# devsisters/libquic

Measured on AMD Instinct MI355X. Metric: FEC XOR encode+recover GiB/s (device-resident) on batched 1350B packet groups, higher is better.
Workload: dtype u8; 1 GPU; 1048576 groups x 10 x 1350 B per GPU: parity encode + single-loss recover (BASELINE configs[1]+[2]); groups_per_gpu=1048576, k=10, L=1350, parallelism=group-shard x1 (no collective)

## Files before the change

libquic_amd/csrc/qfec_kernels.hip:

```cpp
#include "qfec_internal.h"

#include <algorithm>
#include <type_traits>
#include <cstdlib>

namespace qfec {
namespace {

typedef uint32_t u32x4 __attribute__((ext_vector_type(4)));

constexpr uint32_t kMaxPacket = 1452;
constexpr int kBlock = 256;

__device__ __forceinline__ u32x4 ld16(const uint8_t* p) {
  u32x4 v;
  __builtin_memcpy(&v, p, 16);
  return v;
}

template <bool NT>
__device__ __forceinline__ u32x4 ld16t(const uint8_t* p) {
  if constexpr (NT) {
    return __builtin_nontemporal_load(reinterpret_cast<const u32x4*>(p));
  } else {
    return ld16(p);
  }
}

__device__ __forceinline__ void st16(uint8_t* p, u32x4 v) { __builtin_memcpy(p, &v, 16); }

template <bool NT>
__device__ __forceinline__ void st16t(uint8_t* p, u32x4 v) {
  if constexpr (NT) {
    __builtin_nontemporal_store(v, reinterpret_cast<u32x4*>(p));
  } else {
    st16(p, v);
  }
}

__device__ __forceinline__ uint32_t wave_max11(uint32_t v) {
  uint32_t mx = 0;
#pragma unroll
  for (int b = 10; b >= 0; --b) {
    const uint32_t cand = mx | (1u << b);
    if (__ballot(v >= cand) != 0ull) mx = cand;
  }
  return mx;
}

__device__ __forceinline__ bool wave_any(bool p) { return __ballot(p) != 0ull; }

template <int N, bool RECOVER, bool NT>
__device__ __forceinline__ void xor_rows_n(u32x4& acc, const uint8_t* src, uint64_t row_stride,
                                           uint32_t r, uint32_t m, const uint8_t* par) {
  u32x4 v[N];
#pragma unroll
  for (int w = 0; w < N; ++w) {
    const uint8_t* q = (RECOVER && r + (uint32_t)w == m) ? par : src + (uint64_t)(r + w) * row_stride;
    v[w] = ld16t<NT>(q);
  }
#pragma unroll
  for (int w = 0; w < N; ++w) acc ^= v[w];
}

template <int B, bool RECOVER, bool NT>
__device__ __forceinline__ void xor_rows_rt(u32x4& acc, const uint8_t* src, uint64_t row_stride,
                                            uint32_t k, uint32_t m, const uint8_t* par) {
  static_assert(B == 8 || B == 16 || B == 32, "batch of 8, 16 or 32 rows");
  const uint32_t nb = (k + B - 1) / B;
  const uint32_t base = nb ? k / nb : 0u, extra = k - base * nb;
  uint32_t r = 0;
  for (uint32_t b = 0; b < nb; ++b) {
    const uint32_t n = base + (b < extra ? 1u : 0u);
#define QFEC_REM(N)                                                 \
  case N:                                                           \
    xor_rows_n<N, RECOVER, NT>(acc, src, row_stride, r, m, par);    \
    break;
    if (B == 8 || n <= 8u) {
      switch (n) {
        QFEC_REM(1) QFEC_REM(2) QFEC_REM(3) QFEC_REM(4) QFEC_REM(5) QFEC_REM(6) QFEC_REM(7)
        QFEC_REM(8)
        default:
          break;
      }
    } else if constexpr (B >= 16) {
      if (B == 16 || n <= 16u) {
        switch (n) {
          QFEC_REM(9) QFEC_REM(10) QFEC_REM(11) QFEC_REM(12) QFEC_REM(13) QFEC_REM(14)
          QFEC_REM(15) QFEC_REM(16)
          default:
            break;
        }
      } else if constexpr (B == 32) {
        switch (n) {
          QFEC_REM(17) QFEC_REM(18) QFEC_REM(19) QFEC_REM(20) QFEC_REM(21) QFEC_REM(22)
          QFEC_REM(23) QFEC_REM(24) QFEC_REM(25) QFEC_REM(26) QFEC_REM(27) QFEC_REM(28)
          QFEC_REM(29) QFEC_REM(30) QFEC_REM(31) QFEC_REM(32)
          default:
            break;
        }
      }
    }
#undef QFEC_REM
    r += n;
  }
}

template <int KC, bool RECOVER, bool NT, bool SM, bool INPL = false>
__global__ __launch_bounds__(kBlock) void fixed_xor_kernel(FixedArgs a, uint32_t C,
                                                           uint32_t gpb) {
  static_assert(!(INPL && RECOVER), "in place: the encode form over the k rows");
  const uint32_t tid = threadIdx.x;
  const uint32_t gl = tid / C;
  const uint32_t t = tid - gl * C;
  const uint64_t gb = (uint64_t)blockIdx.x * gpb;
  const uint64_t g = gb + gl;
  if constexpr (INPL) {
    const bool on = gl < gpb && g < a.n_groups;
    const uint64_t gg = on ? g : 0;
    const uint32_t off = min(t * 16u, a.L - 16u);
    const uint8_t* src = a.rows + gg * a.group_stride + off;
    const uint32_t k = KC > 0 ? (uint32_t)KC : a.k;
    const uint32_t m = on ? (uint32_t)a.inplace_missing[gg] : 0u;
    u32x4 acc = {0u, 0u, 0u, 0u};
    if constexpr (KC > 0) {
      xor_rows_n<(KC > 0 ? KC : 1), false, NT>(acc, src, a.row_stride, 0, 0, nullptr);
    } else {
      xor_rows_rt<8, false, NT>(acc, src, a.row_stride, k, 0, nullptr);
    }
    __syncthreads();
    if (on && m < k) st16t<NT>(const_cast<uint8_t*>(src) + (uint64_t)m * a.row_stride, acc);
    if (on && m >= k && t == 0) atomicOr(a.err, kErrMissingIndex);
    return;
  }
  uint64_t mw0 = 0, mw1 = 0;
  if constexpr (RECOVER) {
    if constexpr (SM) {
      const uint8_t* mp = a.missing + gb;
      const uint32_t mis = (uint32_t)((uintptr_t)mp & 7u);
      const uint64_t* wp = reinterpret_cast<const uint64_t*>(mp - mis);
      mw0 = wp[0];
      if (gb + 8u - mis < a.n_groups) mw1 = wp[1];
    }
  }
  if (gl >= gpb || g >= a.n_groups) return;
  const uint32_t off = min(t * 16u, a.L - 16u);
  const uint8_t* src = a.rows + g * a.group_stride + off;
  const uint32_t k = KC > 0 ? (uint32_t)KC : a.k;

  u32x4 acc = {0u, 0u, 0u, 0u};
  if constexpr (RECOVER) {
    uint32_t m;
    if constexpr (SM) {
      const uint32_t sh = gl + (uint32_t)((uintptr_t)(a.missing + gb) & 7u);
      m = (uint32_t)((sh < 8u ? mw0 >> (8u * sh) : mw1 >> (8u * (sh - 8u))) & 0xFFu);
    } else {
      m = a.missing[g];
    }
    if (m >= k) {
      if (t == 0) atomicOr(a.err, kErrMissingIndex);
      return;
    }
    const uint8_t* par = a.parity + g * a.parity_stride + off;
    if constexpr (KC > 0) {
#pragma unroll
      for (uint32_t i = 0; i < (uint32_t)KC; ++i) {
        const uint8_t* p = (i == m) ? par : src + i * a.row_stride;
        acc ^= ld16t<NT>(p);
      }
    } else {
      xor_rows_rt<8, true, NT>(acc, src, a.row_stride, k, m, par);
    }
  } else {
    if constexpr (KC > 0) {
#pragma unroll
      for (uint32_t i = 0; i < (uint32_t)KC; ++i) acc ^= ld16t<NT>(src + i * a.row_stride);
    } else {
      xor_rows_rt<8, false, NT>(acc, src, a.row_stride, k, 0, nullptr);
    }
  }
  st16t<NT>(a.out + g * a.out_stride + off, acc);
}

constexpr int kPhSteps = 40;
constexpr int kPhRegSteps = 32;
constexpr uint64_t kPhTimeout = 20000;

__device__ __forceinline__ uint32_t* ph_word(uint32_t* ps, uint32_t i) { return ps + 64u * i; }

__device__ __forceinline__ uint32_t ph_load(uint32_t* w) {
  return __hip_atomic_load(w, __ATOMIC_RELAXED, __HIP_MEMORY_SCOPE_AGENT);
}

constexpr int kPhEarly = 4;

__device__ __forceinline__ uint32_t phase_arrive(uint32_t* ps) {
  return __hip_atomic_fetch_add(ph_word(ps, 1u + (blockIdx.x & 15u)), 1u, __ATOMIC_RELAXED,
                                __HIP_MEMORY_SCOPE_AGENT);
}

__device__ __forceinline__ uint32_t phase_arrive_early(uint32_t* ps) {
  typedef __attribute__((address_space(1))) uint32_t* gptr;
  gptr w = (gptr)ph_word(ps, 1u + (blockIdx.x & 15u));
  asm volatile("" : "+v"(w));
  return __hip_atomic_fetch_add(w, 1u, __ATOMIC_RELAXED, __HIP_MEMORY_SCOPE_AGENT);
}

__device__ __forceinline__ uint32_t phase_full(uint32_t epoch) {
  const uint32_t B = gridDim.x, sub = blockIdx.x & 15u, nsub = (B - sub + 15u) / 16u;
  return epoch * nsub;
}

__device__ __forceinline__ void phase_top(uint32_t* ps) {
  __hip_atomic_fetch_add(ph_word(ps, 0), 1u, __ATOMIC_RELAXED, __HIP_MEMORY_SCOPE_AGENT);
}

__device__ __forceinline__ void phase_arrived(uint32_t* ps, uint32_t epoch, uint32_t old) {
  if (old + 1u == phase_full(epoch)) phase_top(ps);
}

__device__ __forceinline__ bool phase_poll(uint32_t* ps, uint32_t epoch) {
  const uint32_t target = epoch * min(gridDim.x, 16u);
  const uint64_t t0 = wall_clock64();
  while (ph_load(ph_word(ps, 0)) < target) {
    if (wall_clock64() - t0 > kPhTimeout) {
      if (__hip_atomic_fetch_or(ph_word(ps, 18), 1u, __ATOMIC_RELAXED,
                                __HIP_MEMORY_SCOPE_AGENT) == 0u)
        __hip_atomic_fetch_add(ph_word(ps, 19), 1u, __ATOMIC_RELAXED, __HIP_MEMORY_SCOPE_AGENT);
      return true;
    }
    if (ph_load(ph_word(ps, 18)) != 0u) return true;
    __builtin_amdgcn_s_sleep(1);
  }
  return false;
}

template <int E>
__device__ __forceinline__ void phase_wait(uint32_t* ps, uint32_t epoch, uint32_t old, bool late,
                                           bool& gone, uint64_t* T0 = nullptr,
                                           uint64_t* T1 = nullptr) {
  __syncthreads();
  if (T0 && threadIdx.x == 0) *T0 = wall_clock64();
  if constexpr (E == 0) {
    if (threadIdx.x == 0 && ph_load(ph_word(ps, 18)) == 0u) {
      phase_arrived(ps, epoch, phase_arrive(ps));
      gone = phase_poll(ps, epoch);
    }
  } else {
    if (threadIdx.x == 0 && !gone) {
      if (late) phase_arrived(ps, epoch, old);
      gone = phase_poll(ps, epoch);
    }
  }
  if (T1 && threadIdx.x == 0) *T1 = wall_clock64();
  __syncthreads();
}

[[maybe_unused]] __device__ __forceinline__ void phase_meet(uint32_t* ps, uint32_t epoch) {
  bool gone = false;
  phase_wait<0>(ps, epoch, 0u, false, gone);
}

__device__ __forceinline__ void phase_exit(uint32_t* ps, uint32_t* host) {
  __syncthreads();
  if (threadIdx.x == 0 &&
      __hip_atomic_fetch_add(ph_word(ps, 17), 1u, __ATOMIC_RELAXED, __HIP_MEMORY_SCOPE_AGENT) ==
          gridDim.x - 1u) {
    for (uint32_t i = 0; i < 19u; ++i)
      __hip_atomic_store(ph_word(ps, i), 0u, __ATOMIC_RELAXED, __HIP_MEMORY_SCOPE_AGENT);
    if (host)
      __hip_atomic_store(host, ph_load(ph_word(ps, 19)), __ATOMIC_RELAXED,
                         __HIP_MEMORY_SCOPE_SYSTEM);
  }
}

__host__ __device__ constexpr int phase_early(int kc, bool recover, int rs) {
  return recover && rs > 0 && kc >= 24 ? 0 : kPhEarly;
}
#ifdef QFEC_PHASE_TUNE
__device__ uint64_t* g_phase_stamps = nullptr;
#define QFEC_PH_TUNE_TPARAMS , int E = kPhEarly, bool STAMP = false
#else
#define QFEC_PH_TUNE_TPARAMS
#endif
template <int KC, bool RECOVER, int RS = 0, bool INPL = false, int RTB = 32 QFEC_PH_TUNE_TPARAMS>
__global__ __launch_bounds__(kBlock) void phase_xor_kernel(FixedArgs a, uint32_t C, uint32_t gpb,
                                                             uint32_t nphase) {
#ifdef QFEC_PHASE_TUNE
  uint64_t* const stamps =
      STAMP && threadIdx.x == 0 ? g_phase_stamps + (uint64_t)blockIdx.x * nphase * 4u : nullptr;
#else
  constexpr int E = phase_early(KC, RECOVER, RS);
  uint64_t* const stamps = nullptr;
#endif
  static_assert(E >= 0, "arrival E steps before the phase's last step");
  static_assert(!(INPL && RECOVER), "in place: the encode form over the k rows");
  static_assert(kPhSteps <= 64, "recover: bad-step masks are 64 bits");
  static_assert(RS == 0 || (KC > 0 && RS <= 64), "register steps: templated k, 64-bit lane-on mask");
  constexpr bool PF = RECOVER && KC > 0;
  constexpr int TS = kPhSteps + RS;
  const int SP = a.phase_steps != 0u ? min((int)a.phase_steps, TS) : TS;
  const int NL = min(kPhSteps, SP);
  __shared__ u32x4 s_par[kPhSteps][kBlock];
  const uint32_t tid = threadIdx.x, gl = tid / C, t = tid - gl * C;
  const bool lane_on = gl < gpb;
  const uint32_t off = min(t * 16u, a.L - 16u);
  const uint32_t k = KC > 0 ? (uint32_t)KC : a.k;
  const uint64_t B = gridDim.x;
  const int arr = max(SP - E, 0);
  uint32_t ph_old = 0u;
  bool ph_gone = false;
  for (uint32_t p = 0; p < nphase; ++p) {
    int arr_p = arr;
    if constexpr (E > 0) asm volatile("" : "+s"(arr_p));
    const bool ph_on = tid == 0u && !ph_gone;
    const uint32_t ph_full = phase_full(p + 1u);
    auto early = [&](int step) {
      if constexpr (E > 0) {
        if (step == arr_p) {
          if (ph_on) ph_old = phase_arrive_early(a.phase_sync);
        } else if (step == arr_p + 1) {
          if (ph_on && ph_old + 1u == ph_full) phase_top(a.phase_sync);
        }
      }
    };
    const uint64_t base = ((uint64_t)p * (uint64_t)SP * B + blockIdx.x) * gpb + gl;
    uint32_t bad_lo = 0, bad_hi = 0;
    auto gidx = [&](int i) { return base + (uint64_t)i * B * gpb; };
    uint32_t m_reg[RS > 0 && RECOVER ? RS : 1];
    if constexpr (RS > 0 && RECOVER) {
#pragma unroll
      for (int j = 0; j < RS; ++j) {
        const uint64_t g = gidx(kPhSteps + j);
        m_reg[j] = lane_on && g < a.n_groups && kPhSteps + j < SP ? a.missing[g] : 0u;
      }
    }
    constexpr int U = 1;
    uint32_t m_next[U];
    if constexpr (RECOVER) {
#pragma unroll
      for (int u = 0; u < U; ++u) {
        const uint64_t g = gidx(u);
        m_next[u] = lane_on && g < a.n_groups ? a.missing[g] : 0u;
      }
    }
    u32x4 racc[RS > 0 ? RS : 1];
    if constexpr (PF) {
#pragma unroll 1
      for (int i = 0; i < kPhSteps; i += 8) {
        u32x4 w[8];
#pragma unroll
        for (int j = 0; j < 8; ++j) {
          const uint64_t g = gidx(i + j < NL ? i + j : 0);
          const bool on = i + j < NL && lane_on && g < a.n_groups;
          w[j] = ld16t<true>(a.parity + (on ? g : 0) * a.parity_stride + off);
        }
        if (stamps && i == 0) stamps[p * 4u + 3u] = wall_clock64();
#pragma unroll
        for (int j = 0; j < 8; ++j)
          if (i + j < kPhSteps) s_par[i + j][tid] = w[j];
      }
    }
#pragma unroll 1
    for (int i = 0; i < NL; i += U) {
      u32x4 acc[U];
      uint32_t m[U];
      const uint8_t* src[U];
#pragma unroll
      for (int u = 0; u < U; ++u) {
        const uint64_t g = gidx(i + u);
        const bool on = lane_on && g < a.n_groups;
        src[u] = a.rows + (on ? g : 0) * a.group_stride + off;
        acc[u] = u32x4{0u, 0u, 0u, 0u};
        m[u] = k;
        if constexpr (RECOVER) {
          m[u] = m_next[u];
          if (m[u] >= k) {
            if (on) {
              if (i + u < 32) bad_lo |= 1u << (i + u);
              else bad_hi |= 1u << (i + u - 32);
            }
            m[u] = 0u;
          }
        }
      }
#pragma unroll
      for (int u = 0; u < U; ++u) {
        if constexpr (PF) {
          u32x4 v[KC];
#pragma unroll
          for (int r = 0; r + 1 < KC; ++r)
            v[r] = ld16t<true>(src[u] + ((uint32_t)r + ((uint32_t)r >= m[u] ? 1u : 0u)) * a.row_stride);
          v[KC - 1] = u32x4{0u, 0u, 0u, 0u};
          early(i + u);
          acc[u] = s_par[i + u][tid];
#pragma unroll
          for (int r = 0; r < KC; ++r) acc[u] ^= v[r];
        } else if constexpr (KC > 0) {
          u32x4 v[KC];
#pragma unroll
          for (int r = 0; r < KC; ++r) v[r] = ld16t<true>(src[u] + r * a.row_stride);
          if (stamps && i + u == 0) stamps[p * 4u + 3u] = wall_clock64();
          early(i + u);
#pragma unroll
          for (int r = 0; r < KC; ++r) acc[u] ^= v[r];
        } else {
          if (stamps && i + u == 0) stamps[p * 4u + 3u] = wall_clock64();
          early(i + u);
          const uint64_t g = gidx(i + u);
          const uint8_t* par = RECOVER ? a.parity + (lane_on && g < a.n_groups ? g : 0) * a.parity_stride + off
                                       : nullptr;
          xor_rows_rt<RTB, RECOVER, true>(acc[u], src[u], a.row_stride, k, m[u], par);
        }
      }
      if constexpr (RECOVER) {
        if (i + U < NL) {
#pragma unroll
          for (int u = 0; u < U; ++u) {
            const uint64_t g = gidx(i + U + u);
            m_next[u] = lane_on && g < a.n_groups ? a.missing[g] : 0u;
          }
        }
      }
#pragma unroll
      for (int u = 0; u < U; ++u) s_par[i + u][tid] = acc[u];
    }
    uint32_t ron[2] = {0u, 0u};
    bool rbad = false;
    if constexpr (RS > 0) {
      const uint64_t g0r = gidx(kPhSteps);
      const uint8_t* q = a.rows + g0r * a.group_stride + off;
      const uint64_t dq = B * gpb * a.group_stride;
      const uint8_t* qp = RECOVER ? a.parity + g0r * a.parity_stride + off : nullptr;
      const uint64_t dqp = RECOVER ? B * gpb * a.parity_stride : 0u;
      if constexpr (RECOVER) {
#pragma unroll
        for (int j = 0; j < RS; ++j) {
          const uint64_t g = g0r + (uint64_t)j * B * gpb;
          const bool on = lane_on && g < a.n_groups && kPhSteps + j < SP;
          racc[j] = ld16t<true>(a.parity + (on ? g : 0) * a.parity_stride + off);
        }
      }
#pragma unroll
      for (int j = 0; j < RS; ++j) {
        const uint64_t g = g0r + (uint64_t)j * B * gpb;
        bool on = lane_on && g < a.n_groups && kPhSteps + j < SP;
        u32x4 v[KC];
        if constexpr (RECOVER) {
          uint32_t mj = m_reg[j];
          if (mj >= k) {
            rbad = rbad || on;
            on = false;
            mj = 0u;
          }
          const uint8_t* qq = on ? q : a.rows + off;
          v[0] = racc[j];
#pragma unroll
          for (int r = 0; r + 1 < KC; ++r)
            v[r + 1] = ld16t<true>(qq + ((uint32_t)r + ((uint32_t)r >= mj ? 1u : 0u)) * a.row_stride);
        } else {
          const uint8_t* qq = on ? q : a.rows + off;
#pragma unroll
          for (int r = 0; r < KC; ++r) v[r] = ld16t<true>(qq + r * a.row_stride);
        }
        early(kPhSteps + j);
        ron[j / 32] |= on ? 1u << (j % 32) : 0u;
        u32x4 x = v[0];
#pragma unroll
        for (int r = 1; r < KC; ++r) x ^= v[r];
        racc[j] = x;
        q += dq;
        asm volatile("" : "+v"(q) : "v"(x));
        if constexpr (RECOVER) {
          qp += dqp;
          asm volatile("" : "+v"(qp) : "v"(x));
        }
      }
    }
    if constexpr (RECOVER) {
      if (((bad_lo | bad_hi) != 0u || rbad) && t == 0u) atomicOr(a.err, kErrMissingIndex);
    }
    phase_wait<E>(a.phase_sync, p + 1u, ph_old, arr + 1 >= SP, ph_gone, stamps ? stamps + p * 4u : nullptr,
                  stamps ? stamps + p * 4u + 1u : nullptr);
    bool ibad = false;
    auto dst = [&](uint64_t g, bool& on) -> uint8_t* {
      if constexpr (INPL) {
        const uint32_t m = a.inplace_missing[g];
        if (m >= k) {
          ibad = ibad || on;
          on = false;
        }
        return const_cast<uint8_t*>(a.rows) + g * a.group_stride + (uint64_t)m * a.row_stride + off;
      } else {
        return a.out + g * a.out_stride + off;
      }
    };
#pragma unroll 4
    for (int i = 0; i < kPhSteps; ++i) {
      const uint64_t g = gidx(i);
      const uint32_t skip = RECOVER ? ((i < 32 ? bad_lo >> i : bad_hi >> (i - 32)) & 1u) : 0u;
      bool on = lane_on && g < a.n_groups && !skip && i < NL;
      uint8_t* d = dst(on ? g : 0, on);
      if (on) st16t<true>(d, s_par[i][tid]);
    }
    if constexpr (RS > 0) {
#pragma unroll
      for (int j = 0; j < RS; ++j) {
        const uint64_t g = gidx(kPhSteps + j);
        bool on = ((ron[j / 32] >> (j % 32)) & 1u) != 0u;
        uint8_t* d = dst(on ? g : 0, on);
        if (on) st16t<true>(d, racc[j]);
      }
    }
    if constexpr (INPL) {
      if (ibad && t == 0u) atomicOr(a.err, kErrMissingIndex);
    }
    if (stamps) stamps[p * 4u + 2u] = wall_clock64();
  }
  phase_exit(a.phase_sync, a.phase_host);
}

template <bool RECOVER>
__global__ __launch_bounds__(kBlock) void fixed_small_kernel(FixedArgs a) {
  const uint64_t e = (uint64_t)blockIdx.x * kBlock + threadIdx.x;
  const uint64_t g = e / a.L;
  const uint32_t j = (uint32_t)(e - g * a.L);
  if (g >= a.n_groups) return;
  uint8_t acc = 0;
  const uint8_t* src = a.rows + g * a.group_stride + j;
  if (RECOVER) {
    const uint32_t m = a.missing[g];
    if (m >= a.k) {
      if (j == 0) atomicOr(a.err, kErrMissingIndex);
      return;
    }
    acc = a.parity[g * a.parity_stride + j];
    for (uint32_t i = 0; i < a.k; ++i)
      if (i != m) acc ^= src[i * a.row_stride];
  } else {
    for (uint32_t i = 0; i < a.k; ++i) acc ^= src[i * a.row_stride];
  }
  if (a.inplace_missing) {
    const uint32_t m = a.inplace_missing[g];
    if (m >= a.k) {
      if (j == 0) atomicOr(a.err, kErrMissingIndex);
      return;
    }
    const_cast<uint8_t*>(src)[(uint64_t)m * a.row_stride] = acc;
    return;
  }
  a.out[g * a.out_stride + j] = acc;
}

constexpr int kTurnWaves = kReviveTile / 64;
constexpr int kRvScanBlock = 1024;

__device__ __forceinline__ uint32_t lane_id() {
  return __builtin_amdgcn_mbcnt_hi(~0u, __builtin_amdgcn_mbcnt_lo(~0u, 0u));
}

__device__ __forceinline__ uint32_t lane_read(uint32_t x, uint32_t src) {
  return (uint32_t)__builtin_amdgcn_ds_bpermute((int)(src << 2), (int)x);
}

__device__ __forceinline__ uint32_t wave_incl_scan(uint32_t x, uint32_t lane) {
#pragma unroll
  for (int d = 1; d < 64; d <<= 1) {
    const uint32_t y = lane_read(x, lane >= (uint32_t)d ? lane - (uint32_t)d : lane);
    if (lane >= (uint32_t)d) x += y;
  }
  return x;
}

template <int WAVES>
__device__ __forceinline__ uint32_t block_excl_scan(uint32_t x, uint32_t lane, uint32_t wv,
                                                    uint32_t* s_w, uint32_t& total) {
  const uint32_t incl = wave_incl_scan(x, lane);
  if (lane == 63u) s_w[wv] = incl;
  __syncthreads();
  uint32_t base = 0, tot = 0;
#pragma unroll
  for (int w = 0; w < WAVES; ++w) {
    const uint32_t v = s_w[w];
    base += (uint32_t)w < wv ? v : 0u;
    tot += v;
  }
  total = tot;
  __syncthreads();
  return base + incl - x;
}

template <typename Get, typename Put>
__device__ __forceinline__ uint64_t tile_scan(uint64_t n, uint32_t* s_w, Get get, Put put) {
  const uint32_t tid = threadIdx.x, lane = tid & 63u, wave = tid >> 6;
  uint64_t base = 0;
  for (uint64_t t0 = 0; t0 < n; t0 += kRvScanBlock) {
    const uint64_t i = t0 + tid;
    uint32_t tot;
    const uint32_t before =
        block_excl_scan<kRvScanBlock / 64>(i < n ? get(i) : 0u, lane, wave, s_w, tot);
    if (i < n) put(i, base + before);
    base += tot;
  }
  return base;
}
__device__ __forceinline__ uint32_t tile_scan_in_place(uint32_t* v, uint64_t n, uint32_t* s_w) {
  return (uint32_t)tile_scan(
      n, s_w, [=](uint64_t i) { return v[i]; }, [=](uint64_t i, uint64_t x) { v[i] = (uint32_t)x; });
}

__device__ __forceinline__ uint32_t wave_sum(uint32_t v) {
#pragma unroll
  for (int d = 32; d >= 1; d >>= 1) v += __shfl_xor(v, d);
  return v;
}

template <int CH>
__device__ __forceinline__ uint32_t block_sum(const uint32_t (&c)[CH], uint32_t lane,
                                              uint32_t wave, uint32_t* s_w) {
  if (lane == 0u) {
#pragma unroll
    for (int ch = 0; ch < CH; ++ch) s_w[wave * CH + ch] = c[ch];
  }
  __syncthreads();
  const uint32_t ch = min(lane, (uint32_t)(CH - 1));
  uint32_t t = 0;
#pragma unroll
  for (int w = 0; w < kTurnWaves; ++w) t += s_w[w * CH + ch];
  __syncthreads();
  return t;
}
__device__ __forceinline__ uint32_t block_sum(uint32_t c, uint32_t lane, uint32_t wave,
                                              uint32_t* s_w) {
  const uint32_t one[1] = {c};
  return block_sum(one, lane, wave, s_w);
}

__device__ __forceinline__ uint32_t ballot_rank(uint64_t b) {
  return __builtin_amdgcn_mbcnt_hi((uint32_t)(b >> 32),
                                   __builtin_amdgcn_mbcnt_lo((uint32_t)b, 0u));
}

__device__ __forceinline__ uint32_t block_ballot_rank(uint64_t b, uint32_t lane, uint32_t wave,
                                                      uint32_t* s_w, uint32_t& total) {
  if (lane == 0u) s_w[wave] = (uint32_t)__popcll(b);
  __syncthreads();
  uint32_t r = ballot_rank(b), tot = 0;
#pragma unroll
  for (int w = 0; w < kTurnWaves; ++w) {
    const uint32_t v = s_w[w];
    r += (uint32_t)w < wave ? v : 0u;
    tot += v;
  }
  total = tot;
  __syncthreads();
  return r;
}
__device__ __forceinline__ uint32_t block_ballot_rank(uint64_t b, uint32_t lane, uint32_t wave,
                                                      uint32_t* s_w) {
  uint32_t total;
  return block_ballot_rank(b, lane, wave, s_w, total);
}

struct LaneRun {
  bool head;
  uint32_t first, end;
};
__device__ __forceinline__ LaneRun lane_runs(bool eligible, bool same, uint32_t lane) {
  LaneRun r;
  r.head = eligible && (lane == 0u || !same);
  const uint64_t heads = __ballot(r.head), enders = heads | ~__ballot(eligible);
  const uint32_t m_lo = lane < 32u ? (2u << lane) - 1u : 0xFFFFFFFFu;
  const uint32_t m_hi = lane < 32u ? 0u : (2u << (lane - 32u)) - 1u;
  const uint32_t h_lo = (uint32_t)heads & m_lo, h_hi = (uint32_t)(heads >> 32) & m_hi;
  const uint32_t e_lo = (uint32_t)enders & ~m_lo, e_hi = (uint32_t)(enders >> 32) & ~m_hi;
  r.first = h_hi ? 63u - (uint32_t)__builtin_clz(h_hi)
                 : (h_lo ? 31u - (uint32_t)__builtin_clz(h_lo) : 0u);
  r.end = e_lo ? (uint32_t)__builtin_ctz(e_lo)
               : (e_hi ? 32u + (uint32_t)__builtin_ctz(e_hi) : 64u);
  return r;
}
static_assert(kReviveTile % 64 == 0 && kRvScanBlock % 64 == 0, "whole waves");

constexpr uint32_t kGroupComplete = 0, kGroupRevived = 1, kGroupUnrevivable = 2;

__device__ __forceinline__ uint32_t revive_classify(const uint8_t* mp, uint32_t k, uint32_t& m) {
  uint32_t miss, first, fec;
  if (k < 64u) {
    const uint32_t nb = k / 8u + 1u;
    uint32_t lo = 0, hi = 0;
#pragma unroll
    for (uint32_t j = 0; j < 8u; ++j) {
      const uint32_t b = j < nb ? (uint32_t)mp[j] : 0u;
      if (j < 4u) lo |= b << (8u * j);
      else hi |= b << (8u * (j - 4u));
    }
    const uint32_t lom = k >= 32u ? 0xFFFFFFFFu : (1u << k) - 1u;
    const uint32_t him = k > 32u ? (1u << (k - 32u)) - 1u : 0u;
    const uint32_t zl = ~lo & lom, zh = ~hi & him;
    miss = __popc(zl) + __popc(zh);
    first = zl ? (uint32_t)__builtin_ctz(zl) : 32u + (zh ? (uint32_t)__builtin_ctz(zh) : 0u);
    fec = k < 32u ? (lo >> k) & 1u : (hi >> (k - 32u)) & 1u;
  } else {
    miss = 0;
    first = 0;
    const uint32_t nfull = k / 8u, rem = k % 8u;
    for (uint32_t b = 0; b < nfull; ++b) {
      const uint32_t z = ~(uint32_t)mp[b] & 0xFFu;
      if (z != 0u && miss == 0u) first = 8u * b + (uint32_t)__builtin_ctz(z);
      miss += __popc(z);
    }
    const uint32_t last = mp[nfull];
    const uint32_t z = ~last & ((1u << rem) - 1u);
    if (z != 0u && miss == 0u) first = 8u * nfull + (uint32_t)__builtin_ctz(z);
    miss += __popc(z);
    fec = (last >> rem) & 1u;
  }
  m = 0xFFu;
  if (miss == 0u) return kGroupComplete;
  if (miss == 1u && fec != 0u) {
    m = first;
    return kGroupRevived;
  }
  return kGroupUnrevivable;
}

__device__ __forceinline__ bool revive_group_k(const ReviveArgs& a, uint64_t, uint32_t& k) {
  k = a.k;
  return true;
}
__device__ __forceinline__ bool revive_group_k(const ReviveRaggedArgs& a, uint64_t g,
                                               uint32_t& k) {
  k = a.grp_ptr[g + 1] - a.grp_ptr[g];
  return k >= 1u && k <= 255u && (uint64_t)(k / 8u + 1u) <= a.map_stride;
}
__device__ __forceinline__ void revive_bad_group(const ReviveArgs&, uint64_t) {}
__device__ __forceinline__ void revive_bad_group(const ReviveRaggedArgs& a, uint64_t) {
  atomicOr(a.err, kErrGroupSize);
}
__device__ __forceinline__ uint64_t revive_emit_group(const ReviveArgs&, uint64_t, uint32_t) {
  return 0ull;
}
__device__ __forceinline__ uint64_t revive_emit_group(const ReviveRaggedArgs&, uint64_t,
                                                      uint32_t) {
  return 0ull;
}

__device__ __forceinline__ uint32_t close_slot(const CloseArgs& a, uint64_t g) {
  return a.slot ? a.slot[g] : (uint32_t)g;
}
__device__ __forceinline__ bool close_k_ok(const CloseArgs& a, uint32_t k) {
  return k >= 1u && (uint64_t)(k / 8u + 1u) <= a.map_stride;
}
__device__ __forceinline__ bool revive_group_k(const CloseArgs& a, uint64_t g, uint32_t& k) {
  k = a.group_k[g];
  return close_slot(a, g) < a.n_slots && close_k_ok(a, k);
}
__device__ __forceinline__ void revive_bad_group(const CloseArgs& a, uint64_t g) {
  if (close_slot(a, g) >= a.n_slots) atomicOr(a.err, kErrMissingIndex);
  if (!close_k_ok(a, a.group_k[g])) atomicOr(a.err, kErrGroupSize);
}
template <typename Args>
__device__ __forceinline__ const uint8_t* revive_map(const Args& a, uint64_t g) {
  return a.received + g * a.map_stride;
}

__device__ __forceinline__ bool revive_group_k(const TrackedCloseArgs& a, uint64_t g,
                                               uint32_t& k) {
  const uint32_t s = close_slot(a, g);
  k = 0;
  if (s >= a.n_slots) return false;
  k = a.group_k[s];
  return close_k_ok(a, k) && a.acc_len[s] != 0;
}
__device__ __forceinline__ void revive_bad_group(const TrackedCloseArgs& a, uint64_t g) {
  const uint32_t s = close_slot(a, g);
  if (s >= a.n_slots) atomicOr(a.err, kErrMissingIndex);
  else if (!close_k_ok(a, a.group_k[s])) atomicOr(a.err, kErrGroupSize);
// ... 3358 lines not shown
```

Before: 6107 GiB/s.

## Add cross-step row-load lookahead to phase recover kernel, pack missing indices

Adds a templated lookahead depth D that issues the first D row loads of the next group before finishing the current group's XOR, so that load latency overlaps across steps in the recover path. With the default kPhAhead = 0 this path is compiled out. Separately, the per-step missing indices for the register steps are packed four per 32-bit register to cut register use. Loads in the register-step path switch to global-address-space nontemporal loads, and the missing-index reads become unconditional loads from a clamped index. The changes add code complexity and, when D is enabled, register pressure from the held rows.

```diff
diff --git a/libquic_amd/csrc/qfec_kernels.hip b/libquic_amd/csrc/qfec_kernels.hip
--- a/libquic_amd/csrc/qfec_kernels.hip
+++ b/libquic_amd/csrc/qfec_kernels.hip
@@ -25,6 +25,11 @@
   } else {
     return ld16(p);
   }
+}
+
+__device__ __forceinline__ u32x4 ld16gt(const uint8_t* p) {
+  typedef const __attribute__((address_space(1))) u32x4* gptr;
+  return __builtin_nontemporal_load((gptr)p);
 }
 
 __device__ __forceinline__ void st16(uint8_t* p, u32x4 v) { __builtin_memcpy(p, &v, 16); }
@@ -277,9 +282,13 @@
 __host__ __device__ constexpr int phase_early(int kc, bool recover, int rs) {
   return recover && rs > 0 && kc >= 24 ? 0 : kPhEarly;
 }
+constexpr int kPhAhead = 0;
+__host__ __device__ constexpr int phase_ahead(int da, int kc, bool recover, int rs) {
+  return !recover || kc < 2 || (rs > 0 && kc >= 24) ? 0 : da < kc - 1 ? da : kc - 1;
+}
 #ifdef QFEC_PHASE_TUNE
 __device__ uint64_t* g_phase_stamps = nullptr;
-#define QFEC_PH_TUNE_TPARAMS , int E = kPhEarly, bool STAMP = false
+#define QFEC_PH_TUNE_TPARAMS , int E = kPhEarly, bool STAMP = false, int DA = kPhAhead
 #else
 #define QFEC_PH_TUNE_TPARAMS
 #endif
@@ -291,8 +300,10 @@
       STAMP && threadIdx.x == 0 ? g_phase_stamps + (uint64_t)blockIdx.x * nphase * 4u : nullptr;
 #else
   constexpr int E = phase_early(KC, RECOVER, RS);
+  constexpr int DA = kPhAhead;
   uint64_t* const stamps = nullptr;
 #endif
+  constexpr int D = phase_ahead(DA, KC, RECOVER, RS);
   static_assert(E >= 0, "arrival E steps before the phase's last step");
   static_assert(!(INPL && RECOVER), "in place: the encode form over the k rows");
   static_assert(kPhSteps <= 64, "recover: bad-step masks are 64 bits");
@@ -327,14 +338,24 @@
     const uint64_t base = ((uint64_t)p * (uint64_t)SP * B + blockIdx.x) * gpb + gl;
     uint32_t bad_lo = 0, bad_hi = 0;
     auto gidx = [&](int i) { return base + (uint64_t)i * B * gpb; };
-    uint32_t m_reg[RS > 0 && RECOVER ? RS : 1];
+    constexpr int MPK = KC >= 24 ? 1 : 4;
+    uint32_t m_pk[RS > 0 && RECOVER ? (RS + MPK - 1) / MPK : 1];
     if constexpr (RS > 0 && RECOVER) {
+      uint32_t mv[RS];
 #pragma unroll
       for (int j = 0; j < RS; ++j) {
         const uint64_t g = gidx(kPhSteps + j);
-        m_reg[j] = lane_on && g < a.n_groups && kPhSteps + j < SP ? a.missing[g] : 0u;
-      }
-    }
+        mv[j] = a.missing[lane_on && g < a.n_groups && kPhSteps + j < SP ? g : 0];
+      }
+#pragma unroll
+      for (int j = 0; j < RS; ++j) {
+        if (j % MPK == 0) m_pk[j / MPK] = mv[j];
+        else m_pk[j / MPK] |= mv[j] << (8 * (j % MPK));
+      }
+    }
+    auto m_reg = [&](int j) {
+      return MPK == 1 ? m_pk[j] : (m_pk[j / MPK] >> (8 * (j % MPK))) & 0xFFu;
+    };
     constexpr int U = 1;
     uint32_t m_next[U];
     if constexpr (RECOVER) {
@@ -361,72 +382,143 @@
           if (i + j < kPhSteps) s_par[i + j][tid] = w[j];
       }
     }
+    uint32_t ron[2] = {0u, 0u};
+    bool rbad = false;
+    constexpr int DN = D > 0 ? D : 1;
+    [[maybe_unused]] u32x4 hd[DN];
+    [[maybe_unused]] uint32_t m_c = 0u;
+    [[maybe_unused]] const uint8_t* src_c = nullptr;
+    [[maybe_unused]] auto row_c = [&](int r) {
+      return src_c + ((uint32_t)r + ((uint32_t)r >= m_c ? 1u : 0u)) * a.row_stride;
+    };
+    [[maybe_unused]] auto open_lds = [&](int s, uint32_t m, u32x4 after) {
+      const uint64_t g = gidx(s);
+      const bool on = lane_on && g < a.n_groups;
+      if (m >= k) {
+        if (on) {
+          if (s < 32) bad_lo |= 1u << s;
+          else bad_hi |= 1u << (s - 32);
+        }
+        m = 0u;
+      }
+      m_c = m;
+      src_c = a.rows + (on ? g : 0) * a.group_stride + off;
+      asm volatile("" : "+v"(src_c) : "v"(after));
+#pragma unroll
+      for (int r = 0; r < D; ++r) hd[r] = ld16gt(row_c(r));
+    };
+    [[maybe_unused]] auto open_reg = [&](int j, const uint8_t* q, u32x4 after) {
+      const uint64_t g = gidx(kPhSteps + j);
+      bool on = lane_on && g < a.n_groups && kPhSteps + j < SP;
+      uint32_t m = m_reg(j);
+      if (m >= k) {
+        rbad = rbad || on;
+        on = false;
+        m = 0u;
+      }
+      ron[j / 32] |= on ? 1u << (j % 32) : 0u;
+      m_c = m;
+      src_c = on ? q : a.rows + off;
+      asm volatile("" : "+v"(src_c) : "v"(after));
+#pragma unroll
+      for (int r = 0; r < D; ++r) hd[r] = ld16gt(row_c(r));
+    };
+    if constexpr (D > 0) {
+      auto lost = [&](int s) {
+        const uint64_t g = gidx(s);
+        const bool on = lane_on && g < a.n_groups && s < NL;
+        const uint32_t mv = a.missing[on ? g : 0];
+        return on ? mv : 0u;
+      };
+      uint32_t m_n1 = lost(1);
+      open_lds(0, m_next[0], u32x4{0u, 0u, 0u, 0u});
 #pragma unroll 1
-    for (int i = 0; i < NL; i += U) {
-      u32x4 acc[U];
-      uint32_t m[U];
-      const uint8_t* src[U];
-#pragma unroll
-      for (int u = 0; u < U; ++u) {
-        const uint64_t g = gidx(i + u);
-        const bool on = lane_on && g < a.n_groups;
-        src[u] = a.rows + (on ? g : 0) * a.group_stride + off;
-        acc[u] = u32x4{0u, 0u, 0u, 0u};
-        m[u] = k;
-        if constexpr (RECOVER) {
-          m[u] = m_next[u];
-          if (m[u] >= k) {
-            if (on) {
-              if (i + u < 32) bad_lo |= 1u << (i + u);
-              else bad_hi |= 1u << (i + u - 32);
+      for (int i = 0; i < NL; ++i) {
+        u32x4 v[KC];
+#pragma unroll
+        for (int r = D; r + 1 < KC; ++r) v[r] = ld16gt(row_c(r));
+        __builtin_amdgcn_sched_barrier(0);
+        u32x4 acc = s_par[i][tid];
+#pragma unroll
+        for (int r = 0; r < D; ++r) acc ^= hd[r];
+        const uint32_t m_n2 = lost(i + 2);
+        if (i + 1 < NL) {
+          open_lds(i + 1, m_n1, acc);
+        } else if constexpr (RS > 0) {
+          open_reg(0, a.rows + gidx(kPhSteps) * a.group_stride + off, acc);
+        }
+        m_n1 = m_n2;
+        early(i);
+#pragma unroll
+        for (int r = D; r + 1 < KC; ++r) acc ^= v[r];
+        s_par[i][tid] = acc;
+      }
+    } else {
+#pragma unroll 1
+      for (int i = 0; i < NL; i += U) {
+        u32x4 acc[U];
+        uint32_t m[U];
+        const uint8_t* src[U];
+#pragma unroll
+        for (int u = 0; u < U; ++u) {
+          const uint64_t g = gidx(i + u);
+          const bool on = lane_on && g < a.n_groups;
+          src[u] = a.rows + (on ? g : 0) * a.group_stride + off;
+          acc[u] = u32x4{0u, 0u, 0u, 0u};
+          m[u] = k;
+          if constexpr (RECOVER) {
+            m[u] = m_next[u];
+            if (m[u] >= k) {
+              if (on) {
+                if (i + u < 32) bad_lo |= 1u << (i + u);
+                else bad_hi |= 1u << (i + u - 32);
+              }
+              m[u] = 0u;
             }
-            m[u] = 0u;
           }
         }
-      }
-#pragma unroll
-      for (int u = 0; u < U; ++u) {
-        if constexpr (PF) {
-          u32x4 v[KC];
-#pragma unroll
-          for (int r = 0; r + 1 < KC; ++r)
-            v[r] = ld16t<true>(src[u] + ((uint32_t)r + ((uint32_t)r >= m[u] ? 1u : 0u)) * a.row_stride);
-          v[KC - 1] = u32x4{0u, 0u, 0u, 0u};
-          early(i + u);
-          acc[u] = s_par[i + u][tid];
-#pragma unroll
-          for (int r = 0; r < KC; ++r) acc[u] ^= v[r];
-        } else if constexpr (KC > 0) {
-          u32x4 v[KC];
-#pragma unroll
-          for (int r = 0; r < KC; ++r) v[r] = ld16t<true>(src[u] + r * a.row_stride);
-          if (stamps && i + u == 0) stamps[p * 4u + 3u] = wall_clock64();
-          early(i + u);
-#pragma unroll
-          for (int r = 0; r < KC; ++r) acc[u] ^= v[r];
-        } else {
-          if (stamps && i + u == 0) stamps[p * 4u + 3u] = wall_clock64();
-          early(i + u);
-          const uint64_t g = gidx(i + u);
-          const uint8_t* par = RECOVER ? a.parity + (lane_on && g < a.n_groups ? g : 0) * a.parity_stride + off
-                                       : nullptr;
-          xor_rows_rt<RTB, RECOVER, true>(acc[u], src[u], a.row_stride, k, m[u], par);
-        }
-      }
-      if constexpr (RECOVER) {
-        if (i + U < NL) {
-#pragma unroll
-          for (int u = 0; u < U; ++u) {
-            const uint64_t g = gidx(i + U + u);
-            m_next[u] = lane_on && g < a.n_groups ? a.missing[g] : 0u;
+#pragma unroll
+        for (int u = 0; u < U; ++u) {
+          if constexpr (PF) {
+            u32x4 v[KC];
+#pragma unroll
+            for (int r = 0; r + 1 < KC; ++r)
+              v[r] = ld16t<true>(src[u] + ((uint32_t)r + ((uint32_t)r >= m[u] ? 1u : 0u)) * a.row_stride);
+            v[KC - 1] = u32x4{0u, 0u, 0u, 0u};
+            early(i + u);
+            acc[u] = s_par[i + u][tid];
+#pragma unroll
+            for (int r = 0; r < KC; ++r) acc[u] ^= v[r];
+          } else if constexpr (KC > 0) {
+            u32x4 v[KC];
+#pragma unroll
+            for (int r = 0; r < KC; ++r) v[r] = ld16t<true>(src[u] + r * a.row_stride);
+            if (stamps && i + u == 0) stamps[p * 4u + 3u] = wall_clock64();
+            early(i + u);
+#pragma unroll
+            for (int r = 0; r < KC; ++r) acc[u] ^= v[r];
+          } else {
+            if (stamps && i + u == 0) stamps[p * 4u + 3u] = wall_clock64();
+            early(i + u);
+            const uint64_t g = gidx(i + u);
+            const uint8_t* par = RECOVER ? a.parity + (lane_on && g < a.n_groups ? g : 0) * a.parity_stride + off
+                                         : nullptr;
+            xor_rows_rt<RTB, RECOVER, true>(acc[u], src[u], a.row_stride, k, m[u], par);
           }
         }
-      }
-#pragma unroll
-      for (int u = 0; u < U; ++u) s_par[i + u][tid] = acc[u];
-    }
-    uint32_t ron[2] = {0u, 0u};
-    bool rbad = false;
+        if constexpr (RECOVER) {
+          if (i + U < NL) {
+#pragma unroll
+            for (int u = 0; u < U; ++u) {
+              const uint64_t g = gidx(i + U + u);
+              m_next[u] = lane_on && g < a.n_groups ? a.missing[g] : 0u;
+            }
+          }
+        }
+#pragma unroll
+        for (int u = 0; u < U; ++u) s_par[i + u][tid] = acc[u];
+      }
+    }
     if constexpr (RS > 0) {
       const uint64_t g0r = gidx(kPhSteps);
       const uint8_t* q = a.rows + g0r * a.group_stride + off;
@@ -441,39 +533,60 @@
           racc[j] = ld16t<true>(a.parity + (on ? g : 0) * a.parity_stride + off);
         }
       }
-#pragma unroll
-      for (int j = 0; j < RS; ++j) {
-        const uint64_t g = g0r + (uint64_t)j * B * gpb;
-        bool on = lane_on && g < a.n_groups && kPhSteps + j < SP;
-        u32x4 v[KC];
-        if constexpr (RECOVER) {
-          uint32_t mj = m_reg[j];
-          if (mj >= k) {
-            rbad = rbad || on;
-            on = false;
-            mj = 0u;
+      if constexpr (D > 0) {
+#pragma unroll
+        for (int j = 0; j < RS; ++j) {
+          u32x4 v[KC];
+#pragma unroll
+          for (int r = D; r + 1 < KC; ++r) v[r] = ld16gt(row_c(r));
+          __builtin_amdgcn_sched_barrier(0);
+          u32x4 x = racc[j];
+#pragma unroll
+          for (int r = 0; r < D; ++r) x ^= hd[r];
+          if (j + 1 < RS) open_reg(j + 1, q + dq, x);
+          early(kPhSteps + j);
+#pragma unroll
+          for (int r = D; r + 1 < KC; ++r) x ^= v[r];
+          racc[j] = x;
+          q += dq;
+          asm volatile("" : "+v"(q) : "v"(x));
+          if (j + 1 < RS) src_c = (ron[(j + 1) / 32] >> ((j + 1) % 32)) & 1u ? q : a.rows + off;
+        }
+      } else {
+#pragma unroll
+        for (int j = 0; j < RS; ++j) {
+          const uint64_t g = g0r + (uint64_t)j * B * gpb;
+          bool on = lane_on && g < a.n_groups && kPhSteps + j < SP;
+          u32x4 v[KC];
+          if constexpr (RECOVER) {
+            uint32_t mj = m_reg(j);
+            if (mj >= k) {
+              rbad = rbad || on;
+              on = false;
+              mj = 0u;
+            }
+            const uint8_t* qq = on ? q : a.rows + off;
+            v[0] = racc[j];
+#pragma unroll
+            for (int r = 0; r + 1 < KC; ++r)
+              v[r + 1] = ld16gt(qq + ((uint32_t)r + ((uint32_t)r >= mj ? 1u : 0u)) * a.row_stride);
+          } else {
+            const uint8_t* qq = on ? q : a.rows + off;
+#pragma unroll
+            for (int r = 0; r < KC; ++r) v[r] = ld16gt(qq + r * a.row_stride);
           }
-          const uint8_t* qq = on ? q : a.rows + off;
-          v[0] = racc[j];
-#pragma unroll
-          for (int r = 0; r + 1 < KC; ++r)
-            v[r + 1] = ld16t<true>(qq + ((uint32_t)r + ((uint32_t)r >= mj ? 1u : 0u)) * a.row_stride);
-        } else {
-          const uint8_t* qq = on ? q : a.rows + off;
-#pragma unroll
-          for (int r = 0; r < KC; ++r) v[r] = ld16t<true>(qq + r * a.row_stride);
-        }
-        early(kPhSteps + j);
-        ron[j / 32] |= on ? 1u << (j % 32) : 0u;
-        u32x4 x = v[0];
-#pragma unroll
-        for (int r = 1; r < KC; ++r) x ^= v[r];
-        racc[j] = x;
-        q += dq;
-        asm volatile("" : "+v"(q) : "v"(x));
-        if constexpr (RECOVER) {
-          qp += dqp;
-          asm volatile("" : "+v"(qp) : "v"(x));
+          early(kPhSteps + j);
+          ron[j / 32] |= on ? 1u << (j % 32) : 0u;
+          u32x4 x = v[0];
+#pragma unroll
+          for (int r = 1; r < KC; ++r) x ^= v[r];
+          racc[j] = x;
+          q += dq;
+          asm volatile("" : "+v"(q) : "v"(x));
+          if constexpr (RECOVER) {
+            qp += dqp;
+            asm volatile("" : "+v"(qp) : "v"(x));
+          }
         }
       }
     }
```

Result: no change. 6109 GiB/s (median of 6 runs) (+0.0%).
